# gabinsane/multimodal-vae-comparison

Measured on AMD Instinct MI355X. Metric: training samples/sec, MoPoE CdSprites+ L2 (fwd+bwd+Adam), higher is better.
Workload: dtype f32; 1 GPU; configs[1]: MoPoE, CdSprites+ L2 shapes, CNN2 image tower + TxtTransformer text tower, n_latents=32, batch=128/GPU, T=32; Adam(amsgrad) lr 1e-4, beta 1, train mode (dropout on); global_batch=128, parallelism=dp1, settle_steps=40

## Files before the change

### include/mmvae_hip.h

```cpp
#ifndef MMVAE_HIP_H
#define MMVAE_HIP_H

#include <stddef.h>
#include <stdint.h>

#ifdef __cplusplus
extern "C" {
#endif

typedef void* mmvae_stream_t;

enum {
  MMVAE_OK = 0,
  MMVAE_ERR_ARG = 1,
  MMVAE_ERR_UNSUPPORTED = 2,
  MMVAE_ERR_LAUNCH = 3
};

enum { MMVAE_ACT_NONE = 0, MMVAE_ACT_SILU = 1, MMVAE_ACT_RELU = 2, MMVAE_ACT_GELU = 3 };
enum {
  MMVAE_EP_NONE = 0,
  MMVAE_EP_RELU = 1,
  MMVAE_EP_MUL_RELU_MASK = 2,
  MMVAE_EP_MUL_SILU_GRAD = 3,
// ... 25 lines not shown
                                 const mmvae_dropout_t* drop, mmvae_stream_t stream);

int mmvae_ffn32_supported(int d_model, int FF);
int mmvae_proj32_ln_fwd(const float* x, const float* w, const float* b, const float* r, const float* gamma, const float* beta,
                        float* y, float* xhat, float* rstd, int M, const mmvae_dropout_t* drop, mmvae_stream_t stream);
int mmvae_ffn32_bwd_parts(int M, int FF);
size_t mmvae_ffn32_bwd_rowlen(int FF);
int mmvae_ffn32_fwd(const float* x, const float* w1, const float* b1, const float* w2, const float* b2, float* y, int M,
                    int FF, const mmvae_dropout_t* drop, mmvae_stream_t stream);
int mmvae_ffn32_bwd(const float* x, const float* dy, const float* w1, const float* b1, const float* w2, float* dx,
                    float* ws, int M, int FF, const mmvae_dropout_t* drop, mmvae_stream_t stream);
size_t mmvae_ffn32_wsplit_bytes(int FF);
size_t mmvae_ffn32_rsplit_bytes(int M);
int mmvae_ffn32_prep_weights(const float* w1, const float* w2, void* wsplit, int FF, mmvae_stream_t stream);
int mmvae_ffn32_prep_weights_many(const float* const* w1, const float* const* w2, void* const* wsplit, int n, int FF,
                                  mmvae_stream_t stream);
int mmvae_ffn32_fwd_b16(const float* x, const void* wsplit, const float* b1, const float* b2, float* y, int M, int FF,
                        const mmvae_dropout_t* drop, mmvae_stream_t stream);
int mmvae_ffn32_fwd_b16_ln(const float* x, const void* wsplit, const float* b1, const float* b2, const float* r,
                           const float* gamma, const float* beta, float* y, float* xhat, float* rstd, int M, int FF,
                           const mmvae_dropout_t* drop, const mmvae_dropout_t* ln_drop, mmvae_stream_t stream);
int mmvae_ffn32_bwd_b16(const float* x, const float* dy, const void* wsplit, const float* b1, float* dx, float* ws,
                        void* rsplit, const float* dx_add, int M, int FF, const mmvae_dropout_t* drop,
                        mmvae_stream_t stream);

int mmvae_version(void);
const char* mmvae_arch(void);


int mmvae_conv2d_k4s2_fwd(const float* x, const float* w, const float* bias, const float* aux, float* y,
                          int B, int Cin, int Cout, int Hin, int in_act, int ep_mode, mmvae_stream_t stream);

int mmvae_conv2d_k4s2_dgrad(const float* dy, const float* w, const float* aux, float* dx,
                            int B, int Cin, int Cout, int Hout, int ep_mode, mmvae_stream_t stream);

int mmvae_conv2d_k4s2_wgrad(const float* dy, const float* x, float* dw, float* db, float* ws,
                            int B, int Cin, int Cout, int Hout, int x_act, int accumulate, mmvae_stream_t stream);

int mmvae_convT2d_k4s2_fwd(const float* x, const float* w, const float* bias, const float* aux, float* y,
                           int B, int Cin, int Cout, int Hin, int in_act, int ep_mode, mmvae_stream_t stream);

int mmvae_convT2d_k4s2_dgrad(const float* dy, const float* w, const float* aux, float* dx,
                             int B, int Cin, int Cout, int Hin, int ep_mode, mmvae_stream_t stream);

int mmvae_convT2d_k4s2_wgrad(const float* x, const float* dy, float* dw, float* db, float* ws,
                             int B, int Cin, int Cout, int Hin, int x_act, int accumulate, mmvae_stream_t stream);

size_t mmvae_conv_wgrad_ws_floats(int B, int Csmall, int Clarge, int Hsmall);

int mmvae_conv2d_k4s2_bwd(const float* dy, const float* x, const float* w, float* dx, float* dw, float* db, float* ws,
                          int B, int Cin, int Cout, int Hout, int x_act, int accumulate, mmvae_stream_t stream);
int mmvae_convT2d_k4s2_bwd(const float* dy, const float* x, const float* w, float* dx, float* dw, float* db, float* ws,
                           int B, int Cin, int Cout, int Hin, int x_act, int accumulate, mmvae_stream_t stream);
int mmvae_convT3_bce_seeded(const float* x, const float* w, const float* bias, const float* target, float* row,
                            float* dlogit, float* part, unsigned* ticket, int B, int in_act, float seed,
                            mmvae_stream_t stream);
int mmvae_convT3_bce_strips(int B);
int mmvae_conv_plan(int split_bf16);

int mmvae_gemm_f32(const float* A, const float* Bm, const float* bias, const float* aux, float* C,
                   float* a_rowsum, float* ws, int M, int N, int K, long sam, long sak, long sbk, long sbn,
                   long ldc, int a_act, int b_act, int ep_mode, int accumulate, int splitk,
                   mmvae_stream_t stream);
size_t mmvae_gemm_ws_floats(int M, int N, int splitk);
int mmvae_gemm_splits(int M, int N, int K, int splitk);
int mmvae_gemm_b16_set(int on);
int mmvae_bias_group_add(float* y, const float* bias, int rows, int C, int G, mmvae_stream_t stream);
size_t mmvae_bias_group_ws_floats(int rows, int C);
int mmvae_bias_group_parts(int rows);
int mmvae_bias_group_grad(const float* dy, float* db, float* ws, int rows, int C, int G, int accumulate,
                          mmvae_stream_t stream);

int mmvae_linear_fwd(const float* x, const float* w, const float* b, float* aux, float* y, int M, int N, int K,
                     long ldx, int x_act, int ep_mode, mmvae_stream_t stream);
int mmvae_linear_bwd_data(const float* dy, const float* w, const float* aux, float* dx, int M, int N, int K,
                          int ep_mode, int accumulate, mmvae_stream_t stream);
int mmvae_linear_bwd_weight(const float* dy, const float* x, float* dw, float* db, float* ws, int M, int N, int K,
                            long ldx, int x_act, int accumulate, mmvae_stream_t stream);
size_t mmvae_linear_bwd_weight_ws_floats(int M, int N, int K);
#define MMVAE_WGRAD_BATCH_MAX 8
typedef struct {
  const float* dy; const float* x; float* dw; float* db; float* ws;
  int M, N, K; long ldx; int x_act, accumulate;
} mmvae_wgrad_job_t;
int mmvae_linear_bwd_weight_batch(const mmvae_wgrad_job_t* jobs, int n_jobs, mmvae_stream_t stream);
typedef struct {
  const float* dy; const float* x; float* ws;
  int M, N, K;
} mmvae_txt_wgrad_job_t;
int mmvae_txt_wgrad(const mmvae_txt_wgrad_job_t* jobs, int n_jobs, mmvae_stream_t stream);
int mmvae_txt_wgrad_splits(int M, int N, int K);
size_t mmvae_txt_wgrad_ws_floats(int M, int N, int K);
int mmvae_txt_wgrad_supported(int M, int N, int K);
int mmvae_linear_bwd(const float* dy, const float* x, const float* w, const float* aux, float* dx, float* dw,
                     float* db, float* ws, int M, int N, int K, long ldx, int x_act, int ep_mode, int accumulate,
                     mmvae_stream_t stream);
size_t mmvae_linear_bwd_ws_floats(int M, int N, int K);

int mmvae_head_softmax_fwd(float* h, int B, int D, mmvae_stream_t stream);
int mmvae_head_softmax_bwd(const float* h, float* dh, int B, int D, mmvae_stream_t stream);

#define MMVAE_MAX_EXPERTS 8
typedef struct {
  const float* mu[MMVAE_MAX_EXPERTS];
  const float* lv[MMVAE_MAX_EXPERTS];
  const float* eps[MMVAE_MAX_EXPERTS];
// ... 476 lines not shown
```

### multimodal_vae_comparison_amd/hipops.py

```python
import ctypes
import os

import torch

_HERE = os.path.dirname(os.path.abspath(__file__))
LIB_PATH = os.path.join(_HERE, "libmmvae_hip.so")
_lib = None

c_p = ctypes.c_void_p
c_i = ctypes.c_int
c_l = ctypes.c_long
c_f = ctypes.c_float
c_u = ctypes.c_uint
c_sz = ctypes.c_size_t

MAX_EXPERTS = 8

ACT_NONE, ACT_SILU, ACT_RELU, ACT_GELU = 0, 1, 2, 3
EP_NONE, EP_RELU, EP_MUL_RELU_MASK, EP_MUL_SILU_GRAD, EP_GELU, EP_MUL_GELU_GRAD, EP_SIGMOID_CLAMP, EP_SIGMOID, EP_ADD_AUX = range(9)

_ERR = {1: "invalid argument", 2: "unsupported shape", 3: "kernel launch failed"}


class PoeFwdArgs(ctypes.Structure):
# ... 68 lines not shown


class RcDgrad(ctypes.Structure):
    _fields_ = [("G", c_p), ("Y", c_p), ("pqr", c_p), ("w", c_p), ("add", c_p), ("add_tbl", c_p), ("mask", c_i),
                ("mY", c_p), ("mmean", c_p), ("msc", c_p), ("mbeta", c_p), ("out", c_p), ("ws", c_p), ("tile_ticket", c_p),
                ("row_map", c_p), ("M", c_i), ("Min", c_i), ("Cin", c_i), ("Cout", c_i), ("T", c_i), ("nstat", c_i), ("g", RcGeom),
                ("st", RcStat * 2)]


class RcWgrad(ctypes.Structure):
    _fields_ = [("G", c_p), ("Y", c_p), ("pqr", c_p), ("x", c_p), ("xmean", c_p), ("xsc", c_p), ("xbeta", c_p), ("tbl", c_p),
                ("dw", c_p), ("ws", c_p), ("counter", c_p), ("M", c_i), ("Cin", c_i), ("Cout", c_i), ("T", c_i), ("pre", c_i),
                ("accumulate", c_i)]


RC_MAX_JOBS = 8


class RcJob(ctypes.Structure):
    _fields_ = [("kind", c_i), ("f", RcFwd), ("d", RcDgrad), ("w", RcWgrad)]


c_dp = ctypes.POINTER(Dropout)
DROPOUT_SLOTS = 16

SIGNATURES = {
    "mmvae_version": (c_i, []),
    "mmvae_arch": (ctypes.c_char_p, []),
    "mmvae_conv2d_k4s2_fwd": (c_i, [c_p] * 5 + [c_i] * 6 + [c_p]),
    "mmvae_conv2d_k4s2_dgrad": (c_i, [c_p] * 4 + [c_i] * 5 + [c_p]),
    "mmvae_conv2d_k4s2_wgrad": (c_i, [c_p] * 5 + [c_i] * 6 + [c_p]),
    "mmvae_convT2d_k4s2_fwd": (c_i, [c_p] * 5 + [c_i] * 6 + [c_p]),
    "mmvae_convT2d_k4s2_dgrad": (c_i, [c_p] * 4 + [c_i] * 5 + [c_p]),
    "mmvae_convT2d_k4s2_wgrad": (c_i, [c_p] * 5 + [c_i] * 6 + [c_p]),
    "mmvae_conv_wgrad_ws_floats": (c_sz, [c_i] * 4),
    "mmvae_conv2d_k4s2_bwd": (c_i, [c_p] * 7 + [c_i] * 6 + [c_p]),
    "mmvae_convT2d_k4s2_bwd": (c_i, [c_p] * 7 + [c_i] * 6 + [c_p]),
    "mmvae_gemm_f32": (c_i, [c_p] * 7 + [c_i] * 3 + [c_l] * 5 + [c_i] * 5 + [c_p]),
    "mmvae_gemm_ws_floats": (c_sz, [c_i] * 3),
    "mmvae_gemm_splits": (c_i, [c_i] * 4),
    "mmvae_bias_group_add": (c_i, [c_p, c_p, c_i, c_i, c_i, c_p]),
    "mmvae_bias_group_grad": (c_i, [c_p, c_p, c_p, c_i, c_i, c_i, c_i, c_p]),
    "mmvae_bias_group_ws_floats": (c_sz, [c_i, c_i]),
    "mmvae_bias_group_parts": (c_i, [c_i]),
    "mmvae_linear_fwd": (c_i, [c_p] * 5 + [c_i] * 3 + [c_l] + [c_i] * 2 + [c_p]),
    "mmvae_gemm_b16_set": (c_i, [c_i]),
    "mmvae_attn_t_bwd_set": (c_i, [c_i]),
    "mmvae_linear_bwd_data": (c_i, [c_p] * 4 + [c_i] * 5 + [c_p]),
    "mmvae_linear_bwd_weight": (c_i, [c_p] * 5 + [c_i] * 3 + [c_l] + [c_i] * 2 + [c_p]),
    "mmvae_linear_bwd_weight_ws_floats": (c_sz, [c_i] * 3),
    "mmvae_linear_bwd_weight_batch": (c_i, [c_p, c_i, c_p]),
    "mmvae_txt_layer_plan": (c_i, [c_i] * 3),
    "mmvae_conv_plan": (c_i, [c_i]),
    "mmvae_convT3_bce_seeded": (c_i, [c_p] * 8 + [c_i, c_i, c_f, c_p]),
    "mmvae_convT3_bce_strips": (c_i, [c_i]),
    "mmvae_txt_wgrad": (c_i, [c_p, c_i, c_p]),
    "mmvae_txt_wgrad_splits": (c_i, [c_i] * 3),
    "mmvae_txt_wgrad_ws_floats": (c_sz, [c_i] * 3),
    "mmvae_txt_wgrad_supported": (c_i, [c_i] * 3),
    "mmvae_input_pipe_create": (c_i, [c_p, c_p, c_sz]),
    "mmvae_input_pipe_destroy": (c_i, [c_p]),
    "mmvae_input_pipe_prefetch": (c_i, [c_p, c_p]),
    "mmvae_input_pipe_commit": (c_i, [c_p, c_p, c_i, c_p, c_p]),
    "mmvae_linear_bwd": (c_i, [c_p] * 8 + [c_i] * 3 + [c_l] + [c_i] * 3 + [c_p]),
    "mmvae_linear_bwd_ws_floats": (c_sz, [c_i] * 3),
    "mmvae_head_softmax_fwd": (c_i, [c_p, c_i, c_i, c_p]),
    "mmvae_head_softmax_bwd": (c_i, [c_p, c_p, c_i, c_i, c_p]),
    "mmvae_poe_reparam_kl_fwd": (c_i, [ctypes.POINTER(PoeFwdArgs), c_p, c_p, c_p, c_i, c_i, c_i, c_u, c_i, c_i, c_i,
                                       c_i, c_p, c_p]),
    "mmvae_poe_reparam_kl_bwd": (c_i, [ctypes.POINTER(PoeBwdArgs), c_p, c_p, c_p, c_p, c_p, c_i, c_i, c_i, c_u, c_i, c_i,
                                       c_i, c_i, c_i, c_p]),
    "mmvae_poe_reparam_kl_bwd_acc": (c_i, [ctypes.POINTER(PoeBwdArgs), c_p, c_p, c_p, c_p, c_p, c_i, c_i, c_i, c_u, c_i,
                                           c_i, c_i, c_i, c_i, c_u, c_p]),
    "mmvae_poe_ws_floats": (c_sz, [c_i, c_i]),
    "mmvae_bce_rowsum_fwd": (c_i, [c_p] * 3 + [c_i] * 3 + [c_p]),
    "mmvae_bce_sigmoid_clamp_bwd": (c_i, [c_p] * 4 + [c_i] * 3 + [c_p]),
    "mmvae_bce_rowsum_bwd": (c_i, [c_p] * 4 + [c_i] * 2 + [c_p]),
    "mmvae_sigmoid_clamp_bwd": (c_i, [c_p] * 3 + [c_l] + [c_p]),
    "mmvae_bce_elem_fwd": (c_i, [c_p] * 3 + [c_l] + [c_p]),
    "mmvae_bce_rowsum_seeded": (c_i, [c_p] * 3 + [c_f] + [c_p] + [c_i] * 2 + [c_p]),
    "mmvae_ce_over_time_seeded": (c_i, [c_p] * 3 + [c_f] + [c_p] + [c_i] * 3 + [c_p]),
    "mmvae_lprob_elem_fwd": (c_i, [c_p] * 3 + [c_l, c_l, c_f, c_i, c_p]),
    "mmvae_lprob_elem_bwd": (c_i, [c_p] * 4 + [c_l, c_l, c_f, c_i, c_p]),
    "mmvae_optimal_sigma_elem_fwd": (c_i, [c_p] * 5 + [c_l, c_p]),
    "mmvae_optimal_sigma_elem_bwd": (c_i, [c_p] * 6 + [c_l, c_p]),
    "mmvae_pointwise_rowsum_fwd": (c_i, [c_p] * 3 + [c_i] * 4 + [c_p]),
    "mmvae_pointwise_rowsum_bwd": (c_i, [c_p] * 4 + [c_i] * 4 + [c_p]),
    "mmvae_pointwise_elem": (c_i, [c_p] * 4 + [c_l, c_i, c_p]),
    "mmvae_ce_over_time_fwd": (c_i, [c_p] * 4 + [c_i] * 4 + [c_p]),
    "mmvae_ce_over_time_bwd": (c_i, [c_p] * 5 + [c_i] * 4 + [c_p]),
    "mmvae_lincomb_rows_fwd": (c_i, [c_p, ctypes.POINTER(c_f), c_p, c_i, c_i, c_i, c_p]),
    "mmvae_lincomb_rows_bwd": (c_i, [c_p, ctypes.POINTER(c_f), c_p, c_i, c_i, c_i, c_p]),
    "mmvae_expand_image_u8": (c_i, [c_p, c_p, c_l, c_p]),
    "mmvae_expand_text_tokens": (c_i, [c_p] * 4 + [c_i] * 3 + [c_p]),
    "mmvae_randn": (c_i, [c_p, c_l, c_p, c_p]),
    "mmvae_debug_timestamp": (c_i, [c_p, c_p]),
    "mmvae_debug_spin": (c_i, [c_p, ctypes.c_longlong, c_p]),
    "mmvae_conv2d_generic_fwd": (c_i, [c_p] * 5 + [c_i] * 10 + [c_p]),
    "mmvae_conv2d_generic_dgrad": (c_i, [c_p] * 4 + [c_i] * 9 + [c_p]),
    "mmvae_conv2d_generic_wgrad": (c_i, [c_p] * 4 + [c_i] * 10 + [c_p]),
    "mmvae_convT2d_generic_fwd": (c_i, [c_p] * 5 + [c_i] * 10 + [c_p]),
    "mmvae_convT2d_generic_dgrad": (c_i, [c_p] * 4 + [c_i] * 9 + [c_p]),
    "mmvae_convT2d_generic_wgrad": (c_i, [c_p] * 4 + [c_i] * 10 + [c_p]),
    "mmvae_sigmoid_fwd": (c_i, [c_p, c_p, c_l, c_p]),
    "mmvae_sigmoid_bwd": (c_i, [c_p, c_p, c_p, c_l, c_p]),
    "mmvae_lprob_rowsum_fwd": (c_i, [c_p, c_p, c_p, c_i, c_i, c_i, c_f, c_i, c_i, c_i, c_p]),
# ... 234 lines not shown
```

### multimodal_vae_comparison_amd/models/decoders.py

```python
import numpy as np
import torch
import torch.nn as nn

from .. import hipops as H
from .. import ops
from . import encoders
from .NetworkTypes import NetworkRoles, NetworkTypes
from .encoders import VaeComponent
from .nn_modules import DropoutState, HipLayerNorm, HipLinear, HipSelfAttention, ModuleWrap, PositionalEncoding


class VaeDecoder(VaeComponent):
    def __init__(self, latent_dim, data_dim, latent_private, net_type: NetworkTypes):
        super().__init__(latent_dim, data_dim, latent_private, net_type, NetworkRoles.DECODER)


class HipConvT2d(nn.Module):

    def __init__(self, cin, cout, in_act=H.ACT_NONE, out_ep=H.EP_NONE):
        super().__init__()
        ref = nn.ConvTranspose2d(cin, cout, 4, stride=2, padding=1)
        self.weight, self.bias = ref.weight, ref.bias
        self.in_act, self.out_ep = in_act, out_ep

    def flat_groups(self):
        return [[self.weight, self.bias]]

    def forward(self, x, ep_bwd=True):
        return ops.convT2d_k4s2(x, self.weight, self.bias, self.in_act, self.out_ep, self.weight.grad, self.bias.grad,
                                ep_bwd)


class Dec_CNN(VaeDecoder):

    def __init__(self, latent_dim, data_dim, latent_private):
        super().__init__(latent_dim, data_dim, latent_private, net_type=NetworkTypes.CNN)
        hid, hidden_dim = 32, 512
        self.reshape = (hid, 4, 4)
        self.n_chan = 3
        self.lin1 = ModuleWrap(HipLinear(self.out_dim, hidden_dim, H.ACT_NONE))
        self.lin2 = ModuleWrap(HipLinear(hidden_dim, hidden_dim, H.ACT_RELU))
        self.lin3 = ModuleWrap(HipLinear(hidden_dim, int(np.prod(self.reshape)), H.ACT_RELU))
        self.convT_64 = ModuleWrap(HipConvT2d(hid, hid, H.ACT_RELU))
        self.convT1 = ModuleWrap(HipConvT2d(hid, hid, H.ACT_RELU))
        self.convT2 = ModuleWrap(HipConvT2d(hid, hid, H.ACT_RELU))
        self.convT3 = ModuleWrap(HipConvT2d(hid, self.n_chan, H.ACT_RELU, H.EP_SIGMOID_CLAMP))
        self.register_buffer("_scale", torch.tensor(0.75), persistent=False)

    def forward(self, z):
        z_in = z
        z = z["latents"]
        if z.dim() == 2:
            z = z.unsqueeze(0)
        K, bs = z.shape[0], z.shape[1]
        u = self.lin3(self.lin2(self.lin1(z.reshape(K * bs, -1))))
        u = u.view(bs * K, *self.reshape)
        u3 = self.convT2(self.convT1(self.convT_64(u)))
        tgt = z_in.get("bce_target") if isinstance(z_in, dict) else None
        last = self.convT3.module
        if tgt is not None and ops.convT3_bce_supported(u3, last.weight, tgt):
            rows = ops.convT3_bce(u3, last.weight, last.bias, last.in_act, last.weight.grad, last.bias.grad, tgt)
            rows._bce_rows = True
            return rows, self._scale
        raw = last(u3, ep_bwd=False)
        d = ops.sigmoid_clamp_out(raw)
        d = d.view(*z.size()[:-1], *self.data_dim)
        out = d.squeeze().reshape(-1, *self.data_dim)
        out._bce_src = raw
        return out, self._scale


_ONES = {}


def _ones_mask(bs, T, device):
    key = (bs, T, str(device))
    m = _ONES.get(key)
    if m is None:
        if len(_ONES) >= 16:
            _ONES.clear()
        m = _ONES[key] = torch.ones(bs, T, dtype=torch.bool, device=device)
    return m


class HipTransformerDecoderLayer(nn.Module):

    def __init__(self, d, nhead, ff):
        super().__init__()
        self.self_attn = HipSelfAttention(d, nhead)
        self.multihead_attn = HipSelfAttention(d, nhead)
        self.linear1 = HipLinear(d, ff)
        self.linear2 = HipLinear(ff, d, H.ACT_GELU)
        self.norm1 = HipLayerNorm(d)
        self.norm2 = HipLayerNorm(d)
        self.norm3 = HipLayerNorm(d)

    def fused_params(self):
        a, c = self.self_attn, self.multihead_attn
        return {"in_w": a.in_proj_weight, "in_b": a.in_proj_bias, "out_w": a.out_proj.weight, "out_b": a.out_proj.bias,
                "l1_w": self.linear1.weight, "l1_b": self.linear1.bias, "l2_w": self.linear2.weight,
                "l2_b": self.linear2.bias, "n1_g": self.norm1.weight, "n1_b": self.norm1.bias,
                "n2_g": self.norm2.weight, "n2_b": self.norm2.bias, "n3_g": self.norm3.weight, "n3_b": self.norm3.bias,
                "x_in_w": c.in_proj_weight, "x_in_b": c.in_proj_bias, "x_out_w": c.out_proj.weight,
                "x_out_b": c.out_proj.bias}

    def forward(self, x, mem, mask_u8, ds=None):
        L, _, d = x.shape
        ff, nh = self.linear1.out_features, self.self_attn.nhead
        if encoders.FUSED_TXT_LAYERS and ops.txt_layer_supported(L, d, ff, nh, True):
            p = self.fused_params()
# ... 209 lines not shown
```

### multimodal_vae_comparison_amd/models/encoders.py

```python
import os

import numpy as np
import torch
import torch.nn as nn

from .. import hipops as H
from .. import ops
from .NetworkTypes import NetworkRoles, NetworkTypes
from .nn_modules import DropoutState, HipLayerNorm, HipLinear, HipSelfAttention, ModuleWrap, PositionalEncoding


class VaeComponent(nn.Module):

    def __init__(self, latent_dim, data_dim, latent_private=None, enc_mu_logvar=True,
                 net_type=NetworkTypes.UNSPECIFIED, net_role=NetworkRoles.UNSPECIFIED):
        super().__init__()
        self.net_role = net_role
        self.latent_dim = latent_dim
        self.enc_mu_logvar = enc_mu_logvar
        self.latent_private = latent_private
        self.out_dim = latent_dim + latent_private if latent_private is not None else latent_dim
        self.data_dim = data_dim
        self.net_type = net_type
        self.mu_layer = None
# ... 17 lines not shown
        return [[mu.weight, lv.weight], [mu.bias, lv.bias]]

    def process_output(self, data, in_act=H.ACT_NONE):
        mu_l, lv_l = self._heads()
        if not self.enc_mu_logvar:
            return mu_l(data, in_act)
        packed = self.packed_heads() if data.requires_grad else None
        if packed is not None:
            h = ops.linear(data, packed[0], packed[1], in_act, packed[2], packed[3])
        else:
            h = torch.cat([mu_l(data, in_act), lv_l(data, in_act)], dim=-1)
        return self.finish_heads(h)

    def finish_heads(self, h):
        D = self.out_dim
        if not self.raw_heads:
            h = ops.head_softmax(h)
        return h[:, :D], h[:, D:]

    def packed_heads(self):
        if not self.enc_mu_logvar:
            return None
        mu_l, lv_l = self._heads()
        D = self.out_dim
        w_mu, w_lv, b_mu, b_lv = mu_l.weight, lv_l.weight, mu_l.bias, lv_l.bias
        gw_mu, gw_lv, gb_mu, gb_lv = w_mu.grad, w_lv.grad, b_mu.grad, b_lv.grad
        if not (w_lv.data_ptr() == w_mu.data_ptr() + 4 * w_mu.numel()
                and b_lv.data_ptr() == b_mu.data_ptr() + 4 * b_mu.numel()
                and None not in (gw_mu, gw_lv, gb_mu, gb_lv)
                and gw_lv.data_ptr() == gw_mu.data_ptr() + 4 * w_mu.numel()
                and gb_lv.data_ptr() == gb_mu.data_ptr() + 4 * b_mu.numel()):
            return None
        F = w_mu.shape[1]
        return (torch.as_strided(w_mu.detach(), (2 * D, F), (F, 1)), torch.as_strided(b_mu.detach(), (2 * D,), (1,)),
                torch.as_strided(gw_mu, (2 * D, F), (F, 1)), torch.as_strided(gb_mu, (2 * D,), (1,)))


class VaeEncoder(VaeComponent):
    def __init__(self, latent_dim, data_dim, latent_private, enc_mu_logvar, net_type: NetworkTypes):
        super().__init__(latent_dim, data_dim, latent_private, enc_mu_logvar, net_type, NetworkRoles.ENCODER)


class HipConv2d(nn.Module):

    def __init__(self, cin, cout, in_act=H.ACT_NONE):
        super().__init__()
        ref = nn.Conv2d(cin, cout, 4, stride=2, padding=1)
        self.weight, self.bias = ref.weight, ref.bias
        self.in_act = in_act

    def flat_groups(self):
        return [[self.weight, self.bias]]

    def forward(self, x):
        return ops.conv2d_k4s2(x, self.weight, self.bias, self.in_act, self.weight.grad, self.bias.grad)


class Enc_CNN2(VaeEncoder):

    def __init__(self, latent_dim, data_dim, latent_private, enc_mu_logvar):
        data_dim = (3, 64, 64)
        super().__init__(latent_dim, data_dim, latent_private, enc_mu_logvar, net_type=NetworkTypes.CNN)
        hid = 32
        self.hidden_dim = 512
        self.reshape = (hid, 4, 4)
        self.conv1 = HipConv2d(3, hid, H.ACT_NONE)
        self.conv2 = HipConv2d(hid, hid, H.ACT_SILU)
        self.conv3 = HipConv2d(hid, hid, H.ACT_SILU)
        self.conv4 = HipConv2d(hid, hid, H.ACT_SILU)
        self.lin1 = HipLinear(int(np.prod(self.reshape)), self.hidden_dim, H.ACT_SILU)
        self.init_final_layers(self.hidden_dim)

    def forward(self, x):
        if isinstance(x, dict):
            x = x["data"]
        bs = x.size(0)
        u = self.conv4(self.conv3(self.conv2(self.conv1(x.float()))))
        o5 = self.lin1(u.view(bs, -1))
        return self.process_output(o5)


class HipConv(nn.Module):

    def __init__(self, cin, cout, k, stride, pad, in_act=H.ACT_NONE, transposed=False, out_ep=H.EP_NONE):
        super().__init__()
        ref = (nn.ConvTranspose2d if transposed else nn.Conv2d)(cin, cout, k, stride=stride, padding=pad)
        self.weight, self.bias = ref.weight, ref.bias
        self.cfg = (stride, pad, in_act, transposed, out_ep)

    def flat_groups(self):
        return [[self.weight, self.bias]]

    def forward(self, x, ep_bwd=True):
        stride, pad, in_act, transposed, out_ep = self.cfg
        if transposed:
            return ops.convT2d(x, self.weight, self.bias, stride, pad, in_act, out_ep, self.weight.grad, self.bias.grad,
                               ep_bwd)
        return ops.conv2d(x, self.weight, self.bias, stride, pad, in_act, self.weight.grad, self.bias.grad)


class _HiddenHeads:

    def _heads(self):
        return self.hidden_mu, self.hidden_logvar


class Enc_MNIST(_HiddenHeads, VaeEncoder):

    def __init__(self, latent_dim, data_dim, latent_private, enc_mu_logvar):
        super().__init__(latent_dim, data_dim, latent_private, enc_mu_logvar, net_type=NetworkTypes.FNN)
        self.net_type = "CNN"
        self.hidden_dim = 400
        self.enc = nn.ModuleList([nn.ModuleList([HipLinear(784, self.hidden_dim)]),
                                  nn.ModuleList([HipLinear(self.hidden_dim, self.hidden_dim, H.ACT_RELU)])])
        self.hidden_mu = HipLinear(self.hidden_dim, self.out_dim)
        self.hidden_logvar = HipLinear(self.hidden_dim, self.out_dim)

    def forward(self, x):
        x = x["data"] if isinstance(x, dict) else x
        h = x.reshape(x.shape[0], -1).float()
        h = self.enc[1][0](self.enc[0][0](h))
        return self.process_output(h, H.ACT_RELU)


class Enc_SVHN(_HiddenHeads, VaeEncoder):

    def __init__(self, latent_dim, data_dim, latent_private, enc_mu_logvar):
        super().__init__(latent_dim, data_dim, latent_private, enc_mu_logvar, net_type=NetworkTypes.CNN)
        self.net_type = "CNN"
        self.conv1 = HipConv(3, 32, 4, 2, 1)
# ... 259 lines not shown
```

### multimodal_vae_comparison_amd/ops.py

```python
import bisect
import ctypes
import os

import torch
from torch.autograd import Function

from . import hipops as H

_DACT = {H.ACT_NONE: H.EP_NONE, H.ACT_SILU: H.EP_MUL_SILU_GRAD, H.ACT_RELU: H.EP_MUL_RELU_MASK,
         H.ACT_GELU: H.EP_MUL_GELU_GRAD}


CALLS = [0]


def _call(name, *args):
    CALLS[0] += 1
    H.check(getattr(H.lib(), name)(*args), name)


class GradReducer:

    enabled = True
    tail = None
# ... 369 lines not shown
    return drop.c()


def dropout_advance(state, slot):
    _call("mmvae_dropout_advance", H.ptr(state), int(slot), H.stream())


def dropout_advance_many(states):
    arr = (ctypes.c_void_p * len(states))(*[H.ptr(t) for t in states])
    _call("mmvae_dropout_advance_many", ctypes.cast(arr, ctypes.c_void_p), len(states), H.stream())


def dropout_mask(drop, n):
    out = torch.empty(n, device=drop.state.device)
    _call("mmvae_dropout_mask", drop.c(), H.ptr(out), n, H.stream())
    return out


def _new_like_param(p, g):
    if g is not None:
        return g, 1, None
    t = torch.empty_like(p)
    return t, 0, t


def _grad_dst(w, gw, gb, has_b, n_bias):
    dw, acc_w, ret_w = _new_like_param(w, gw)
    db = ret_b = None
    if has_b:
        db = gb
        if gb is None:
            db = ret_b = torch.empty(n_bias, device=w.device)
    return dw, db, acc_w, ret_w, ret_b


class Conv2dK4S2(Function):

    @staticmethod
    def forward(ctx, x, w, b, in_act, gw, gb):
        x = H.f32c(x)
        B, Cin, Hin, _ = x.shape
        Cout = w.shape[0]
        y = torch.empty(B, Cout, Hin // 2, Hin // 2, device=x.device, dtype=torch.float32)
        _call("mmvae_conv2d_k4s2_fwd", H.ptr(x), H.ptr(w), H.ptr(b), None, H.ptr(y), B, Cin, Cout, Hin, in_act,
              H.EP_NONE, H.stream())
        ctx.save_for_backward(x, w)
        ctx.cfg = (in_act, gw, gb, b is not None)
        return y

    @staticmethod
    def backward(ctx, dy):
        x, w = ctx.saved_tensors
        in_act, gw, gb, has_b = ctx.cfg
        dy = H.f32c(dy)
        B, Cin, Hin, _ = x.shape
        Cout, Hout = w.shape[0], Hin // 2
        dw, db, acc_w, ret_w, ret_b = _grad_dst(w, gw, gb, has_b, Cout)
        nws = H.lib().mmvae_conv_wgrad_ws_floats(B, Cout, Cin, Hout)
        defer = _defer(gw, gb if has_b else gw)
        ws = GradReducer.alloc(nws, x.device) if defer else H.workspace(nws, x.device)
        acc = H.ACC_DEFER if defer else acc_w
        dx = None
        if ctx.needs_input_grad[0]:
            dx = torch.empty_like(x)
            _call("mmvae_conv2d_k4s2_bwd", H.ptr(dy), H.ptr(x), H.ptr(w), H.ptr(dx), H.ptr(dw), H.ptr(db), H.ptr(ws),
                  B, Cin, Cout, Hout, in_act, acc, H.stream())
        else:
            _call("mmvae_conv2d_k4s2_wgrad", H.ptr(dy), H.ptr(x), H.ptr(dw), H.ptr(db), H.ptr(ws), B, Cin, Cout, Hout,
                  in_act, acc, H.stream())
        if defer:
            _conv_segments(ws, dw, db, B, Cout, Cin, Hout, Cout)
        return dx, ret_w, ret_b, None, None, None


class ConvT2dK4S2(Function):

    @staticmethod
    def forward(ctx, x, w, b, in_act, out_ep, gw, gb, ep_bwd=True):
        x = H.f32c(x)
        B, Cin, Hin, _ = x.shape
        Cout = w.shape[1]
        y = torch.empty(B, Cout, 2 * Hin, 2 * Hin, device=x.device, dtype=torch.float32)
        _call("mmvae_convT2d_k4s2_fwd", H.ptr(x), H.ptr(w), H.ptr(b), None, H.ptr(y), B, Cin, Cout, Hin, in_act,
              out_ep, H.stream())
        if not ep_bwd:
            out_ep = H.EP_NONE
        ctx.save_for_backward(x, w, y if out_ep in (H.EP_SIGMOID_CLAMP, H.EP_SIGMOID) else None)
        ctx.cfg = (in_act, out_ep, gw, gb, b is not None)
        return y

    @staticmethod
    def backward(ctx, dy):
        x, w, y = ctx.saved_tensors
        in_act, out_ep, gw, gb, has_b = ctx.cfg
        dy = H.f32c(dy)
        B, Cin, Hin, _ = x.shape
        Cout = w.shape[1]
        if out_ep == H.EP_SIGMOID_CLAMP:
            dl = torch.empty_like(dy)
            _call("mmvae_sigmoid_clamp_bwd", H.ptr(dy), H.ptr(y), H.ptr(dl), dy.numel(), H.stream())
            dy = dl
        elif out_ep == H.EP_SIGMOID:
            dl = torch.empty_like(dy)
            _call("mmvae_sigmoid_bwd", H.ptr(dy), H.ptr(y), H.ptr(dl), dy.numel(), H.stream())
            dy = dl
        dx, ret_w, ret_b = _convT_k4s2_bwd(x, w, dy, in_act, gw, gb, has_b, ctx.needs_input_grad[0])
        return dx, ret_w, ret_b, None, None, None, None, None


def _convT_k4s2_bwd(x, w, dy, in_act, gw, gb, has_b, need_dx):
    B, Cin, Hin, _ = x.shape
    Cout = w.shape[1]
    dw, db, acc_w, ret_w, ret_b = _grad_dst(w, gw, gb, has_b, Cout)
    nws = H.lib().mmvae_conv_wgrad_ws_floats(B, Cin, Cout, Hin)
    defer = _defer(gw, gb if has_b else gw)
    ws = GradReducer.alloc(nws, x.device) if defer else H.workspace(nws, x.device)
    acc = H.ACC_DEFER if defer else acc_w
    dx = None
    if need_dx:
        dx = torch.empty_like(x)
        _call("mmvae_convT2d_k4s2_bwd", H.ptr(dy), H.ptr(x), H.ptr(w), H.ptr(dx), H.ptr(dw), H.ptr(db), H.ptr(ws),
              B, Cin, Cout, Hin, in_act, acc, H.stream())
    else:
        _call("mmvae_convT2d_k4s2_wgrad", H.ptr(x), H.ptr(dy), H.ptr(dw), H.ptr(db), H.ptr(ws), B, Cin, Cout, Hin,
              in_act, acc, H.stream())
    if defer:
        _conv_segments(ws, dw, db, B, Cin, Cout, Hin, Cout)
    return dx, ret_w, ret_b


_T3_SCRATCH = {}


class ConvT3Bce(Function):

    calls = 0

    @staticmethod
    def forward(ctx, x, w, b, in_act, gw, gb, target, cs):
        ConvT3Bce.calls += 1
        x, target = H.f32c(x), H.f32c(target)
        B = x.shape[0]
        dev = x.device
        row = torch.empty(B, device=dev)
        dl = torch.empty(B, 3, 64, 64, device=dev)
        S = H.lib().mmvae_convT3_bce_strips(B)
        part = tick = None
        if S > 1:
            key = (dev.index, H.stream(), B)
            ent = _T3_SCRATCH.get(key)
            if ent is None:
                assert not torch.cuda.is_current_stream_capturing(), \
                    "ConvT3Bce: first call at this batch size inside a graph capture (run one eager warm-up step first)"
                ent = _T3_SCRATCH[key] = (torch.zeros(B * S, device=dev), torch.zeros(B, dtype=torch.int32, device=dev))
            part, tick = ent
        _call("mmvae_convT3_bce_seeded", H.ptr(x), H.ptr(w), H.ptr(b), H.ptr(target), H.ptr(row), H.ptr(dl), H.ptr(part),
              H.ptr(tick), B, in_act, cs.value, H.stream())
        ctx.save_for_backward(x, w, dl)
        ctx.cfg = (in_act, gw, gb, b is not None, cs.seed.data_ptr(), cs.value)
        return row

    @staticmethod
    def backward(ctx, g):
        x, w, dl = ctx.saved_tensors
        in_act, gw, gb, has_b, seed_ptr, seed_value = ctx.cfg
        if g.data_ptr() != seed_ptr:
            dl = dl * (H.f32c(g) / seed_value).view(-1, 1, 1, 1)
        dx, ret_w, ret_b = _convT_k4s2_bwd(x, w, dl, in_act, gw, gb, has_b, ctx.needs_input_grad[0])
        return dx, ret_w, ret_b, None, None, None, None, None


CONVT3_BCE = True


def convT3_bce_supported(x, w, target):
    return (CONVT3_BCE and x.shape[0] >= 256 and ConstSeed.current is not None and ConstSeed.current.value != 0 and
            x.is_cuda and x.dim() == 4 and tuple(x.shape[1:]) == (32, 32, 32) and
            tuple(w.shape) == (32, 3, 4, 4) and target.numel() == x.shape[0] * 3 * 64 * 64 and x.requires_grad)


def convT3_bce(x, w, b, in_act, gw, gb, target):
# ... 2269 lines not shown
```

Baseline: 333,500 samples/s.

## Fuse consecutive small k4s2 conv and convT layer pairs into single kernels

Adds fused HIP kernels that run two back-to-back 32-channel k4s2 conv layers (encoder conv3+conv4) and transposed conv layers (decoder convT_64+convT1) in one launch per image. The intermediate activation stays in LDS for the second layer and is also written out for backward. Backward still runs the two existing per-layer kernels, driven by new autograd Functions. The aim is to cut launch overhead and a global round trip of the intermediate activation. The trade-off is one block per image with heavy register use for weights, which may limit occupancy.

New measurement: 332,800 samples/s. Within noise of the previous version (-0.2%).

```diff
diff --git a/include/mmvae_hip.h b/include/mmvae_hip.h
--- a/include/mmvae_hip.h
+++ b/include/mmvae_hip.h
@@ -101,6 +101,11 @@
                           int B, int Cin, int Cout, int Hout, int x_act, int accumulate, mmvae_stream_t stream);
 int mmvae_convT2d_k4s2_bwd(const float* dy, const float* x, const float* w, float* dx, float* dw, float* db, float* ws,
                            int B, int Cin, int Cout, int Hin, int x_act, int accumulate, mmvae_stream_t stream);
+int mmvae_conv2d_k4s2_pair_fwd(const float* x, const float* w1, const float* b1, const float* w2, const float* b2,
+                               float* mid, float* y, int B, int in_act1, int in_act2, mmvae_stream_t stream);
+int mmvae_convT2d_k4s2_pair_fwd(const float* x, const float* w1, const float* b1, const float* w2, const float* b2,
+                                float* mid, float* y, int B, int in_act1, int in_act2, mmvae_stream_t stream);
+int mmvae_conv_pair_set(int mask);
 int mmvae_convT3_bce_seeded(const float* x, const float* w, const float* bias, const float* target, float* row,
                             float* dlogit, float* part, unsigned* ticket, int B, int in_act, float seed,
                             mmvae_stream_t stream);
diff --git a/multimodal_vae_comparison_amd/csrc/conv_pair.hip b/multimodal_vae_comparison_amd/csrc/conv_pair.hip
--- /dev/null
+++ b/multimodal_vae_comparison_amd/csrc/conv_pair.hip
@@ -0,0 +1,320 @@
+#include "conv_common.hpp"
+#include "conv_pair_args.hpp"
+
+#include <stdlib.h>
+
+namespace {
+
+struct ConvPairArgs {
+  const float *x, *w1, *b1, *w2, *b2;
+  float *mid, *y;
+  int act1, act2;
+};
+
+constexpr int PAIR_C = 32;
+constexpr int PX_RW = 18, PX_CS = PX_RW * PX_RW;
+constexpr int PM_RW = 10, PM_CS = PM_RW * PM_RW;
+constexpr int PT_RW = 6, PT_CS = PT_RW * PT_RW;
+
+__device__ __forceinline__ float pair_act(float v, int act) {
+  return act == MMVAE_ACT_SILU ? dev_silu(v) : act == MMVAE_ACT_RELU ? fmaxf(v, 0.f) : v;
+}
+__device__ __forceinline__ float f4at(const float4& v, int t) { return t == 0 ? v.x : t == 1 ? v.y : t == 2 ? v.z : v.w; }
+
+template <int HW>
+__device__ __forceinline__ void pair_zero_halo(float* __restrict__ s, int tid) {
+  constexpr int RW = HW + 2, NH = 4 * HW + 4;
+  for (int i = tid; i < PAIR_C * NH; i += 256) {
+    const int c = i / NH, j = i - c * NH;
+    int pos;
+    if (j < RW) pos = j;
+    else if (j < 2 * RW) pos = (HW + 1) * RW + (j - RW);
+    else pos = (1 + ((j - 2 * RW) >> 1)) * RW + ((j - 2 * RW) & 1) * (HW + 1);
+    s[c * RW * RW + pos] = 0.f;
+  }
+}
+
+__device__ __forceinline__ void pair_load_w(float4 (&wq)[8][2], const float* __restrict__ wl) {
+#pragma unroll
+  for (int cc = 0; cc < 8; ++cc) {
+    wq[cc][0] = *reinterpret_cast<const float4*>(wl + cc * 16);
+    wq[cc][1] = *reinterpret_cast<const float4*>(wl + cc * 16 + 16 * PAIR_C * 16);
+  }
+}
+template <int CS>
+__device__ __forceinline__ void pair_mfma8(const float* __restrict__ sa, const float4 (&wq)[8][2], f32x4 (&acc)[2]) {
+  float av[2][4];
+#pragma unroll
+  for (int t = 0; t < 4; ++t) av[0][t] = sa[t];
+#pragma unroll
+  for (int cc = 0; cc < 8; ++cc) {
+    if (cc + 1 < 8) {
+#pragma unroll
+      for (int t = 0; t < 4; ++t) av[(cc + 1) & 1][t] = sa[(cc + 1) * CS + t];
+    }
+    __builtin_amdgcn_sched_barrier(0);
+#pragma unroll
+    for (int t = 0; t < 4; ++t) {
+      acc[0] = __builtin_amdgcn_mfma_f32_16x16x4f32(av[cc & 1][t], f4at(wq[cc][0], t), acc[0], 0, 0, 0);
+      acc[1] = __builtin_amdgcn_mfma_f32_16x16x4f32(av[cc & 1][t], f4at(wq[cc][1], t), acc[1], 0, 0, 0);
+    }
+    __builtin_amdgcn_sched_barrier(0);
+  }
+}
+
+__global__ __launch_bounds__(256) void conv_pair_kernel(ConvPairArgs a) {
+  MMVAE_TRACE_STAMP(40);
+  __shared__ __attribute__((aligned(16))) float s_x[PAIR_C * PX_CS];
+  __shared__ __attribute__((aligned(16))) float s_m[PAIR_C * PM_CS];
+  const int tid = threadIdx.x, lane = tid & 63, wave = __builtin_amdgcn_readfirstlane(tid >> 6);
+  const int li = lane & 15, lk = lane >> 4;
+  const size_t b = blockIdx.x;
+
+  const float* wl1 = a.w1 + li * (PAIR_C * 16) + lk * 4;
+  float4 wa[8][2], wb[8][2];
+  pair_load_w(wa, wl1);
+  {
+    const float* xb = a.x + b * (PAIR_C * 256);
+    float4 rv[8];
+#pragma unroll
+    for (int s = 0; s < 8; ++s) rv[s] = *reinterpret_cast<const float4*>(xb + 4 * (tid + 256 * s));
+    pair_zero_halo<16>(s_x, tid);
+    pair_zero_halo<8>(s_m, tid);
+#pragma unroll
+    for (int s = 0; s < 8; ++s) {
+      const int q = tid + 256 * s, c = q >> 6, r = (q >> 2) & 15, c4 = q & 3;
+      float* d = s_x + c * PX_CS + (r + 1) * PX_RW + 1 + 4 * c4;
+      d[0] = pair_act(rv[s].x, a.act1);
+      d[1] = pair_act(rv[s].y, a.act1);
+      d[2] = pair_act(rv[s].z, a.act1);
+      d[3] = pair_act(rv[s].w, a.act1);
+    }
+  }
+  __syncthreads();
+
+  f32x4 acc[2];
+#pragma unroll
+  for (int n = 0; n < 2; ++n) acc[n] = f32x4{0.f, 0.f, 0.f, 0.f};
+  {
+    const int oh = 2 * wave + (li >> 3), ow = li & 7;
+    const float* sa = s_x + (2 * oh + lk) * PX_RW + 2 * ow;
+    pair_load_w(wb, wl1 + 8 * 16);
+    pair_mfma8<PX_CS>(sa, wa, acc);
+    pair_load_w(wa, wl1 + 16 * 16);
+    pair_mfma8<PX_CS>(sa + 8 * PX_CS, wb, acc);
+    pair_load_w(wb, wl1 + 24 * 16);
+    pair_mfma8<PX_CS>(sa + 16 * PX_CS, wa, acc);
+    pair_load_w(wa, a.w2 + li * (PAIR_C * 16) + wave * 8 * 16 + lk * 4);
+    pair_mfma8<PX_CS>(sa + 24 * PX_CS, wb, acc);
+  }
+  {
+    const int oh = 2 * wave + (lk >> 1), ow0 = 4 * (lk & 1);
+#pragma unroll
+    for (int n = 0; n < 2; ++n) {
+      const int o = n * 16 + li;
+      const float bias = a.b1 ? a.b1[o] : 0.f;
+      const float4 v = make_float4(acc[n][0] + bias, acc[n][1] + bias, acc[n][2] + bias, acc[n][3] + bias);
+      *reinterpret_cast<float4*>(a.mid + ((b * PAIR_C + o) * 8 + oh) * 8 + ow0) = v;
+      float* d = s_m + o * PM_CS + (oh + 1) * PM_RW + 1 + ow0;
+      d[0] = pair_act(v.x, a.act2);
+      d[1] = pair_act(v.y, a.act2);
+      d[2] = pair_act(v.z, a.act2);
+      d[3] = pair_act(v.w, a.act2);
+    }
+  }
+  __syncthreads();
+
+#pragma unroll
+  for (int n = 0; n < 2; ++n) acc[n] = f32x4{0.f, 0.f, 0.f, 0.f};
+  pair_mfma8<PM_CS>(s_m + wave * 8 * PM_CS + (2 * (li >> 2) + lk) * PM_RW + 2 * (li & 3), wa, acc);
+  float* red = s_x;
+#pragma unroll
+  for (int n = 0; n < 2; ++n)
+#pragma unroll
+    for (int r = 0; r < 4; ++r) red[((wave * 2 + n) * 4 + r) * 64 + lane] = acc[n][r];
+  __syncthreads();
+  if (tid < 128) {
+    const int n = tid >> 6, o = n * 16 + li;
+    const float bias = a.b2 ? a.b2[o] : 0.f;
+    float v[4];
+#pragma unroll
+    for (int r = 0; r < 4; ++r) {
+      float s = bias;
+#pragma unroll
+      for (int w = 0; w < 4; ++w) s += red[((w * 2 + n) * 4 + r) * 64 + lane];
+      v[r] = s;
+    }
+    *reinterpret_cast<float4*>(a.y + (b * PAIR_C + o) * 16 + 4 * lk) = make_float4(v[0], v[1], v[2], v[3]);
+  }
+}
+
+__device__ __forceinline__ void pairT_load_w(float2 (&wq)[8][2][2], const float* __restrict__ wl) {
+#pragma unroll
+  for (int cc = 0; cc < 8; ++cc)
+#pragma unroll
+    for (int n = 0; n < 2; ++n) {
+      wq[cc][n][0] = *reinterpret_cast<const float2*>(wl + cc * (PAIR_C * 16) + n * 256);
+      wq[cc][n][1] = *reinterpret_cast<const float2*>(wl + cc * (PAIR_C * 16) + n * 256 + 4);
+    }
+}
+__device__ __forceinline__ void pairT_mfma8(const float* __restrict__ sa, const float2 (&wq)[8][2][2],
+                                            f32x4 (&acc)[2][2][2]) {
+  float av[2][2][2];
+  auto load_a = [&](int cc, int buf) {
+#pragma unroll
+    for (int ph = 0; ph < 2; ++ph)
+#pragma unroll
+      for (int pw = 0; pw < 2; ++pw) av[buf][ph][pw] = sa[cc * PM_CS + ph * PM_RW + pw];
+  };
+  load_a(0, 0);
+#pragma unroll
+  for (int cc = 0; cc < 8; ++cc) {
+    if (cc + 1 < 8) load_a(cc + 1, (cc + 1) & 1);
+    __builtin_amdgcn_sched_barrier(0);
+#pragma unroll
+    for (int ph = 0; ph < 2; ++ph)
+#pragma unroll
+      for (int pw = 0; pw < 2; ++pw)
+#pragma unroll
+        for (int n = 0; n < 2; ++n) {
+          const float2 wr = wq[cc][n][1 - ph];
+          acc[n][ph][pw] = __builtin_amdgcn_mfma_f32_16x16x4f32(av[cc & 1][ph][pw], pw ? wr.x : wr.y,
+                                                                acc[n][ph][pw], 0, 0, 0);
+        }
+    __builtin_amdgcn_sched_barrier(0);
+  }
+}
+
+__global__ __launch_bounds__(256) void convT_pair_kernel(ConvPairArgs a) {
+  MMVAE_TRACE_STAMP(41);
+  __shared__ __attribute__((aligned(16))) float s_x[PAIR_C * PT_CS];
+  __shared__ __attribute__((aligned(16))) float s_m[PAIR_C * PM_CS];
+  const int tid = threadIdx.x, lane = tid & 63, wave = __builtin_amdgcn_readfirstlane(tid >> 6);
+  const int li = lane & 15, lk = lane >> 4, ka = lk >> 1, kb = lk & 1;
+  const size_t b = blockIdx.x;
+
+  const int n1 = wave & 1, ph1 = wave >> 1;
+  float2 w1q[PAIR_C];
+  {
+    const float* wl1 = a.w1 + (n1 * 16 + li) * 16 + (1 - ph1 + 2 * ka) * 4 + 2 * kb;
+#pragma unroll
+    for (int c = 0; c < PAIR_C; ++c) w1q[c] = *reinterpret_cast<const float2*>(wl1 + c * (PAIR_C * 16));
+  }
+  const float* wl2 = a.w2 + li * 16 + 2 * ka * 4 + 2 * kb;
+  float2 qa[8][2][2], qb[8][2][2];
+  pairT_load_w(qa, wl2);
+  {
+    float4 rv = make_float4(0.f, 0.f, 0.f, 0.f);
+    if (tid < 128) rv = *reinterpret_cast<const float4*>(a.x + b * (PAIR_C * 16) + 4 * tid);
+    pair_zero_halo<4>(s_x, tid);
+    pair_zero_halo<8>(s_m, tid);
+    if (tid < 128) {
+      float* d = s_x + (tid >> 2) * PT_CS + ((tid & 3) + 1) * PT_RW + 1;
+      d[0] = pair_act(rv.x, a.act1);
+      d[1] = pair_act(rv.y, a.act1);
+      d[2] = pair_act(rv.z, a.act1);
+      d[3] = pair_act(rv.w, a.act1);
+    }
+  }
+  __syncthreads();
+
+  {
+    f32x4 acc1[2];
+#pragma unroll
+    for (int pw = 0; pw < 2; ++pw) acc1[pw] = f32x4{0.f, 0.f, 0.f, 0.f};
+    const float* sa = s_x + ((li >> 2) + ph1 - ka + 1) * PT_RW + ((li & 3) - kb + 1);
+    float av[2][2];
+    av[0][0] = sa[0];
+    av[0][1] = sa[1];
+#pragma unroll
+    for (int c = 0; c < PAIR_C; ++c) {
+      if (c + 1 < PAIR_C) {
+        av[(c + 1) & 1][0] = sa[(c + 1) * PT_CS];
+        av[(c + 1) & 1][1] = sa[(c + 1) * PT_CS + 1];
+      }
+      __builtin_amdgcn_sched_barrier(0);
+      acc1[0] = __builtin_amdgcn_mfma_f32_16x16x4f32(av[c & 1][0], w1q[c].y, acc1[0], 0, 0, 0);
+      acc1[1] = __builtin_amdgcn_mfma_f32_16x16x4f32(av[c & 1][1], w1q[c].x, acc1[1], 0, 0, 0);
+      __builtin_amdgcn_sched_barrier(0);
+    }
+    const int o = n1 * 16 + li, oh = 2 * lk + ph1;
+    const float bias = a.b1 ? a.b1[o] : 0.f;
+    float v[8];
+#pragma unroll
+    for (int r = 0; r < 4; ++r) {
+      v[2 * r] = acc1[0][r] + bias;
+      v[2 * r + 1] = acc1[1][r] + bias;
+    }
+    float* g = a.mid + ((b * PAIR_C + o) * 8 + oh) * 8;
+    *reinterpret_cast<float4*>(g) = make_float4(v[0], v[1], v[2], v[3]);
+    *reinterpret_cast<float4*>(g + 4) = make_float4(v[4], v[5], v[6], v[7]);
+    float* d = s_m + o * PM_CS + (oh + 1) * PM_RW + 1;
+#pragma unroll
+    for (int j = 0; j < 8; ++j) d[j] = pair_act(v[j], a.act2);
+  }
+  __syncthreads();
+
+  f32x4 acc[2][2][2];
+#pragma unroll
+  for (int i = 0; i < 8; ++i) acc[i >> 2][(i >> 1) & 1][i & 1] = f32x4{0.f, 0.f, 0.f, 0.f};
+  {
+    const float* sa = s_m + (2 * wave + (li >> 3) - ka + 1) * PM_RW + ((li & 7) - kb + 1);
+    pairT_load_w(qb, wl2 + 8 * (PAIR_C * 16));
+    pairT_mfma8(sa, qa, acc);
+    pairT_load_w(qa, wl2 + 16 * (PAIR_C * 16));
+    pairT_mfma8(sa + 8 * PM_CS, qb, acc);
+    pairT_load_w(qb, wl2 + 24 * (PAIR_C * 16));
+    pairT_mfma8(sa + 16 * PM_CS, qa, acc);
+    pairT_mfma8(sa + 24 * PM_CS, qb, acc);
+  }
+  const int mh = 2 * wave + (lk >> 1);
+#pragma unroll
+  for (int n = 0; n < 2; ++n) {
+    const int o = n * 16 + li;
+    const float bias = a.b2 ? a.b2[o] : 0.f;
+#pragma unroll
+    for (int ph = 0; ph < 2; ++ph) {
+      float* g = a.y + ((b * PAIR_C + o) * 16 + 2 * mh + ph) * 16 + 8 * (lk & 1);
+      const f32x4 e = acc[n][ph][0], f = acc[n][ph][1];
+      *reinterpret_cast<float4*>(g) = make_float4(e[0] + bias, f[0] + bias, e[1] + bias, f[1] + bias);
+      *reinterpret_cast<float4*>(g + 4) = make_float4(e[2] + bias, f[2] + bias, e[3] + bias, f[3] + bias);
+    }
+  }
+}
+
+int g_conv_pair_mask = -1;
+int conv_pair_mask() {
+  if (g_conv_pair_mask < 0) {
+    const char* e = getenv("MMVAE_CONV_PAIR");
+    g_conv_pair_mask = e ? (atoi(e) & 3) : 3;
+  }
+  return g_conv_pair_mask;
+}
+
+}
+
+extern "C" int mmvae_conv2d_k4s2_pair_fwd(const float* x, const float* w1, const float* b1, const float* w2, const float* b2,
+                                          float* mid, float* y, int B, int in_act1, int in_act2, mmvae_stream_t stream) {
+  const int rc = conv_pair_check_args(x, w1, b1, w2, b2, mid, y, B, in_act1, in_act2);
+  if (rc) return rc;
+  ConvPairArgs a{x, w1, b1, w2, b2, mid, y, in_act1, in_act2};
+  hipLaunchKernelGGL(conv_pair_kernel, dim3(B), dim3(256), 0, (hipStream_t)stream, a);
+  return mmvae_launch_status();
+}
+
+extern "C" int mmvae_convT2d_k4s2_pair_fwd(const float* x, const float* w1, const float* b1, const float* w2, const float* b2,
+                                           float* mid, float* y, int B, int in_act1, int in_act2, mmvae_stream_t stream) {
+  const int rc = conv_pair_check_args(x, w1, b1, w2, b2, mid, y, B, in_act1, in_act2);
+  if (rc) return rc;
+  ConvPairArgs a{x, w1, b1, w2, b2, mid, y, in_act1, in_act2};
+  hipLaunchKernelGGL(convT_pair_kernel, dim3(B), dim3(256), 0, (hipStream_t)stream, a);
+  return mmvae_launch_status();
+}
+
+extern "C" int mmvae_conv_pair_set(int mask) {
+  const int old = conv_pair_mask();
+  if (mask >= 0) g_conv_pair_mask = mask & 3;
+  return old;
+}
+
+MMVAE_TRACE_SETTER(conv_pair)
diff --git a/multimodal_vae_comparison_amd/csrc/conv_pair_args.hpp b/multimodal_vae_comparison_amd/csrc/conv_pair_args.hpp
--- /dev/null
+++ b/multimodal_vae_comparison_amd/csrc/conv_pair_args.hpp
@@ -0,0 +1,17 @@
+#pragma once
+#include <stdint.h>
+
+#include "mmvae_hip.h"
+
+static inline int conv_pair_check_args(const float* x, const float* w1, const float* b1, const float* w2, const float* b2,
+                                       const float* mid, const float* y, int B, int in_act1, int in_act2) {
+  (void)b1;
+  (void)b2;
+  if (!x || !w1 || !w2 || !mid || !y || B <= 0) return MMVAE_ERR_ARG;
+  if ((((uintptr_t)x | (uintptr_t)w1 | (uintptr_t)w2 | (uintptr_t)mid | (uintptr_t)y) & 15) != 0) return MMVAE_ERR_ARG;
+  if (B > (1 << 20)) return MMVAE_ERR_UNSUPPORTED;
+  const int acts[2] = {in_act1, in_act2};
+  for (int a : acts)
+    if (a != MMVAE_ACT_NONE && a != MMVAE_ACT_SILU && a != MMVAE_ACT_RELU) return MMVAE_ERR_UNSUPPORTED;
+  return MMVAE_OK;
+}
diff --git a/multimodal_vae_comparison_amd/hipops.py b/multimodal_vae_comparison_amd/hipops.py
--- a/multimodal_vae_comparison_amd/hipops.py
+++ b/multimodal_vae_comparison_amd/hipops.py
@@ -144,6 +144,9 @@
     "mmvae_linear_bwd_weight_batch": (c_i, [c_p, c_i, c_p]),
     "mmvae_txt_layer_plan": (c_i, [c_i] * 3),
     "mmvae_conv_plan": (c_i, [c_i]),
+    "mmvae_conv2d_k4s2_pair_fwd": (c_i, [c_p] * 7 + [c_i] * 3 + [c_p]),
+    "mmvae_convT2d_k4s2_pair_fwd": (c_i, [c_p] * 7 + [c_i] * 3 + [c_p]),
+    "mmvae_conv_pair_set": (c_i, [c_i]),
     "mmvae_convT3_bce_seeded": (c_i, [c_p] * 8 + [c_i, c_i, c_f, c_p]),
     "mmvae_convT3_bce_strips": (c_i, [c_i]),
     "mmvae_txt_wgrad": (c_i, [c_p, c_i, c_p]),
diff --git a/multimodal_vae_comparison_amd/models/decoders.py b/multimodal_vae_comparison_amd/models/decoders.py
--- a/multimodal_vae_comparison_amd/models/decoders.py
+++ b/multimodal_vae_comparison_amd/models/decoders.py
@@ -26,7 +26,12 @@
     def flat_groups(self):
         return [[self.weight, self.bias]]
 
-    def forward(self, x, ep_bwd=True):
+    def pair_args(self):
+        return self.weight, self.bias, self.in_act, self.weight.grad, self.bias.grad
+
+    def forward(self, x, ep_bwd=True, done=None):
+        if done is not None:
+            return done
         return ops.convT2d_k4s2(x, self.weight, self.bias, self.in_act, self.out_ep, self.weight.grad, self.bias.grad,
                                 ep_bwd)
 
@@ -55,7 +60,8 @@
         K, bs = z.shape[0], z.shape[1]
         u = self.lin3(self.lin2(self.lin1(z.reshape(K * bs, -1))))
         u = u.view(bs * K, *self.reshape)
-        u3 = self.convT2(self.convT1(self.convT_64(u)))
+        o1, o2 = ops.convT2d_k4s2_pair(u, self.convT_64.module.pair_args(), self.convT1.module.pair_args())
+        u3 = self.convT2(self.convT1(self.convT_64(u, done=o1), done=o2))
         tgt = z_in.get("bce_target") if isinstance(z_in, dict) else None
         last = self.convT3.module
         if tgt is not None and ops.convT3_bce_supported(u3, last.weight, tgt):
diff --git a/multimodal_vae_comparison_amd/models/encoders.py b/multimodal_vae_comparison_amd/models/encoders.py
--- a/multimodal_vae_comparison_amd/models/encoders.py
+++ b/multimodal_vae_comparison_amd/models/encoders.py
@@ -93,7 +93,12 @@
     def flat_groups(self):
         return [[self.weight, self.bias]]
 
-    def forward(self, x):
+    def pair_args(self):
+        return self.weight, self.bias, self.in_act, self.weight.grad, self.bias.grad
+
+    def forward(self, x, done=None):
+        if done is not None:
+            return done
         return ops.conv2d_k4s2(x, self.weight, self.bias, self.in_act, self.weight.grad, self.bias.grad)
 
 
@@ -116,7 +121,9 @@
         if isinstance(x, dict):
             x = x["data"]
         bs = x.size(0)
-        u = self.conv4(self.conv3(self.conv2(self.conv1(x.float()))))
+        h = self.conv2(self.conv1(x.float()))
+        o3, o4 = ops.conv2d_k4s2_pair(h, self.conv3.pair_args(), self.conv4.pair_args())
+        u = self.conv4(self.conv3(h, done=o3), done=o4)
         o5 = self.lin1(u.view(bs, -1))
         return self.process_output(o5)
 
diff --git a/multimodal_vae_comparison_amd/ops.py b/multimodal_vae_comparison_amd/ops.py
--- a/multimodal_vae_comparison_amd/ops.py
+++ b/multimodal_vae_comparison_amd/ops.py
@@ -445,25 +445,29 @@
     def backward(ctx, dy):
         x, w = ctx.saved_tensors
         in_act, gw, gb, has_b = ctx.cfg
-        dy = H.f32c(dy)
-        B, Cin, Hin, _ = x.shape
-        Cout, Hout = w.shape[0], Hin // 2
-        dw, db, acc_w, ret_w, ret_b = _grad_dst(w, gw, gb, has_b, Cout)
-        nws = H.lib().mmvae_conv_wgrad_ws_floats(B, Cout, Cin, Hout)
-        defer = _defer(gw, gb if has_b else gw)
-        ws = GradReducer.alloc(nws, x.device) if defer else H.workspace(nws, x.device)
-        acc = H.ACC_DEFER if defer else acc_w
-        dx = None
-        if ctx.needs_input_grad[0]:
-            dx = torch.empty_like(x)
-            _call("mmvae_conv2d_k4s2_bwd", H.ptr(dy), H.ptr(x), H.ptr(w), H.ptr(dx), H.ptr(dw), H.ptr(db), H.ptr(ws),
-                  B, Cin, Cout, Hout, in_act, acc, H.stream())
-        else:
-            _call("mmvae_conv2d_k4s2_wgrad", H.ptr(dy), H.ptr(x), H.ptr(dw), H.ptr(db), H.ptr(ws), B, Cin, Cout, Hout,
-                  in_act, acc, H.stream())
-        if defer:
-            _conv_segments(ws, dw, db, B, Cout, Cin, Hout, Cout)
+        dx, ret_w, ret_b = _conv_k4s2_bwd(x, w, H.f32c(dy), in_act, gw, gb, has_b, ctx.needs_input_grad[0])
         return dx, ret_w, ret_b, None, None, None
+
+
+def _conv_k4s2_bwd(x, w, dy, in_act, gw, gb, has_b, need_dx):
+    B, Cin, Hin, _ = x.shape
+    Cout, Hout = w.shape[0], Hin // 2
+    dw, db, acc_w, ret_w, ret_b = _grad_dst(w, gw, gb, has_b, Cout)
+    nws = H.lib().mmvae_conv_wgrad_ws_floats(B, Cout, Cin, Hout)
+    defer = _defer(gw, gb if has_b else gw)
+    ws = GradReducer.alloc(nws, x.device) if defer else H.workspace(nws, x.device)
+    acc = H.ACC_DEFER if defer else acc_w
+    dx = None
+    if need_dx:
+        dx = torch.empty_like(x)
+        _call("mmvae_conv2d_k4s2_bwd", H.ptr(dy), H.ptr(x), H.ptr(w), H.ptr(dx), H.ptr(dw), H.ptr(db), H.ptr(ws),
+              B, Cin, Cout, Hout, in_act, acc, H.stream())
+    else:
+        _call("mmvae_conv2d_k4s2_wgrad", H.ptr(dy), H.ptr(x), H.ptr(dw), H.ptr(db), H.ptr(ws), B, Cin, Cout, Hout,
+              in_act, acc, H.stream())
+    if defer:
+        _conv_segments(ws, dw, db, B, Cout, Cin, Hout, Cout)
+    return dx, ret_w, ret_b
 
 
 class ConvT2dK4S2(Function):
@@ -520,6 +524,86 @@
     if defer:
         _conv_segments(ws, dw, db, B, Cin, Cout, Hin, Cout)
     return dx, ret_w, ret_b
+
+
+def _pair_forward(ctx, entry, mid_hw, out_hw, x, w1, b1, w2, b2, l1, l2):
+    B = x.shape[0]
+    mid = torch.empty(B, 32, mid_hw, mid_hw, device=x.device, dtype=torch.float32)
+    y = torch.empty(B, 32, out_hw, out_hw, device=x.device, dtype=torch.float32)
+    _call(entry, H.ptr(x), H.ptr(w1), H.ptr(b1), H.ptr(w2), H.ptr(b2), H.ptr(mid), H.ptr(y), B, l1[0], l2[0], H.stream())
+    ctx.save_for_backward(x, w1, mid, w2)
+    ctx.cfg = (l1 + (b1 is not None,), l2 + (b2 is not None,))
+    ctx.mark_non_differentiable(mid)
+    ctx.set_materialize_grads(False)
+    return mid, y
+
+
+def _pair_backward(ctx, layer_bwd, dy):
+    if dy is None:
+        return (None,) * 7
+    x, w1, mid, w2 = ctx.saved_tensors
+    l1, l2 = ctx.cfg
+    dmid, ret_w2, ret_b2 = layer_bwd(mid, w2, H.f32c(dy), *l2, True)
+    dx, ret_w1, ret_b1 = layer_bwd(x, w1, dmid, *l1, ctx.needs_input_grad[0])
+    return dx, ret_w1, ret_b1, ret_w2, ret_b2, None, None
+
+
+class Conv2dK4S2Pair(Function):
+    IN_HW, BIT = 16, 1
+
+    @staticmethod
+    def forward(ctx, x, w1, b1, w2, b2, l1, l2):
+        return _pair_forward(ctx, "mmvae_conv2d_k4s2_pair_fwd", 8, 4, x, w1, b1, w2, b2, l1, l2)
+
+    @staticmethod
+    def backward(ctx, _dmid, dy):
+        return _pair_backward(ctx, _conv_k4s2_bwd, dy)
+
+
+class ConvT2dK4S2Pair(Function):
+    IN_HW, BIT = 4, 2
+
+    @staticmethod
+    def forward(ctx, x, w1, b1, w2, b2, l1, l2):
+        return _pair_forward(ctx, "mmvae_convT2d_k4s2_pair_fwd", 8, 16, x, w1, b1, w2, b2, l1, l2)
+
+    @staticmethod
+    def backward(ctx, _dmid, dy):
+        return _pair_backward(ctx, _convT_k4s2_bwd, dy)
+
+
+CONV_PAIR_MAX_IMAGES = 256
+
+
+def conv_pair_set(mask):
+    return H.lib().mmvae_conv_pair_set(mask)
+
+
+def conv_pair_supported(pair, x, w1, w2):
+    if not conv_pair_set(-1) & pair.BIT:
+        return False
+    if x.dim() != 4 or tuple(x.shape[1:]) != (32, pair.IN_HW, pair.IN_HW) or not 1 <= x.shape[0] <= CONV_PAIR_MAX_IMAGES:
+        return False
+    for t, shape in ((x, x.shape), (w1, (32, 32, 4, 4)), (w2, (32, 32, 4, 4))):
+        if not (t.is_cuda and t.dtype == torch.float32 and tuple(t.shape) == tuple(shape) and t.is_contiguous()
+                and t.data_ptr() % 16 == 0):
+            return False
+    return True
+
+
+def _k4s2_pair(pair, single, x, l1, l2):
+    if conv_pair_supported(pair, x, l1[0], l2[0]):
+        return pair.apply(x, l1[0], l1[1], l2[0], l2[1], tuple(l1[2:]), tuple(l2[2:]))
+    mid = single(x, *l1)
+    return mid, single(mid, *l2)
+
+
+def conv2d_k4s2_pair(x, l1, l2):
+    return _k4s2_pair(Conv2dK4S2Pair, conv2d_k4s2, x, l1, l2)
+
+
+def convT2d_k4s2_pair(x, l1, l2):
+    return _k4s2_pair(ConvT2dK4S2Pair, lambda t, w, b, act, gw, gb: convT2d_k4s2(t, w, b, act, H.EP_NONE, gw, gb), x, l1, l2)
 
 
 _T3_SCRATCH = {}
```
